# Polochon-street/bliss-rs

Measured on AMD Instinct MI355X. Metric: songs/sec (3-min 22 050 Hz f32) at 1/2/4/8 GPU; HBM GB/s vs roofline, higher is better.
Workload: dtype f32; 1 GPU; configs[1]: batch of 1024 synthetic 3969000-sample (3-min) white-noise f32 PCM buffers per GPU, full 23-feature descriptor set (FeaturesVersion 2); songs_per_gpu=1024, songs_total=1024, features=23, parallelism=single GPU

## Files before the change

bliss-rs_amd/csrc/ctx.hpp:

```cpp
#pragma once
#include <hip/hip_runtime.h>
#include <sched.h>

#include <map>
#include <memory>
#include <mutex>
#include <string>
#include <vector>

#include "../../include/blissgpu.h"
#include "internal.hpp"
#include "resample.hpp"
#include "staging_ring.hpp"

namespace bg {

int fail(int code, const char* what, const char* detail);

#define HIP_TRY(expr)                                                                           \
    do {                                                                                        \
        hipError_t e_ = (expr);                                                                 \
        if (e_ != hipSuccess) return ::bg::fail(BLISSGPU_ERR_HIP, #expr, hipGetErrorString(e_)); \
    } while (0)

struct EventPair { hipEvent_t a, b; };

template <typename T>
struct DevBuf {
    T* p = nullptr;
    size_t cap = 0;
    int ensure(size_t n) {
        if (n <= cap) return BLISSGPU_OK;
        if (p) (void)hipFree(p);
        p = nullptr;
        cap = 0;
        size_t want = n + n / 8 + 64;
        hipError_t e = hipMalloc((void**)&p, want * sizeof(T));
        if (e != hipSuccess && want > n) {
            (void)hipGetLastError();
            want = n;
            e = hipMalloc((void**)&p, want * sizeof(T));
        }
        if (e != hipSuccess) {
            (void)hipGetLastError();
            p = nullptr;
            return fail(BLISSGPU_ERR_OOM, "hipMalloc", hipGetErrorString(e));
        }
        cap = want;
        return BLISSGPU_OK;
    }
    void release() { if (p) (void)hipFree(p); p = nullptr; cap = 0; }
};

template <typename T>
struct PinnedBuf {
    T* p = nullptr;
    size_t cap = 0;
    int ensure(size_t n) {
        if (n <= cap) return BLISSGPU_OK;
        if (p) (void)hipHostFree(p);
        p = nullptr;
        cap = 0;
        const size_t want = n + n / 4 + 64;
        hipError_t e = hipHostMalloc((void**)&p, want * sizeof(T), hipHostMallocDefault);
        if (e != hipSuccess) { (void)hipGetLastError(); p = nullptr; return fail(BLISSGPU_ERR_OOM, "hipHostMalloc", hipGetErrorString(e)); }
        cap = want;
        return BLISSGPU_OK;
    }
    void release() { if (p) (void)hipHostFree(p); p = nullptr; cap = 0; }
};

struct ChunkSlot {
    DevBuf<uint8_t> slab;
    DevBuf<uint8_t> desc;
    PinnedBuf<uint8_t> h_desc;
    hipEvent_t ev_start = nullptr, ev_fork = nullptr, ev_stft = nullptr, ev_sel = nullptr, ev_tune = nullptr, ev_sum = nullptr, ev_chroma = nullptr;
    hipEvent_t ev_acf = nullptr, ev_beat = nullptr;
    bool beat_masked = false;
    static constexpr int MAX_PIECES = 8;
    hipEvent_t ev_piece[MAX_PIECES] = {};
    int pieces = 0;
    bg::SongRange piece[MAX_PIECES]{};
    hipEvent_t ev_desc = nullptr;
    hipEvent_t ev_free = nullptr;
    bool used = false;
    bool back_pending = false;
    Batch batch{};
    Workspace ws{};
};

#ifndef FEED_COPY_STREAMS
#define FEED_COPY_STREAMS 2
#endif
#ifndef STAGE_LANES_DEFAULT
#define STAGE_LANES_DEFAULT 4
#endif
#ifndef STAGE_SLABS_DEFAULT
#define STAGE_SLABS_DEFAULT 3
#endif
#ifndef STAGE_SLAB_KIB_DEFAULT
#define STAGE_SLAB_KIB_DEFAULT 4096
#endif
#ifndef STAGE_EVENT_FLAGS
#define STAGE_EVENT_FLAGS (hipEventDisableTiming | hipEventBlockingSync)
#endif
constexpr int N_COPY_STREAMS = FEED_COPY_STREAMS;
#ifndef FEED_BUFFERS
#define FEED_BUFFERS 3
#endif
constexpr int N_FEED_BUFFERS = FEED_BUFFERS;
constexpr uint32_t MAX_SAMPLE_RATE = 768000;
struct FeedSong {
    const void* p;
    uint64_t frames;
    uint32_t rate;
    uint8_t fmt;
    uint8_t channels;
    size_t frame_bytes() const { return (size_t)(fmt == BLISSGPU_SAMPLE_S16 ? 2 : 4) * channels; }
    bool direct() const { return fmt == BLISSGPU_SAMPLE_F32 && channels == 1 && rate == SWR_OUT_RATE; }
};
struct ResampleBank {
    SwrPlan plan;
    float* d_bank = nullptr;
    size_t bytes = 0;
    uint64_t last_use = 0;
};
#ifndef SWR_CACHE_BYTES
#define SWR_CACHE_BYTES (64ull << 20)
#endif

constexpr int MAX_STAGE_LANES = 16;
struct HipStageDev {
    int device;
    hipStream_t* streams;
    std::vector<int> cpus;
    void thread_begin(int) {
        (void)hipSetDevice(device);
        if (!cpus.empty()) {
            cpu_set_t set;
            CPU_ZERO(&set);
            for (int cpu : cpus)
                if (cpu >= 0 && cpu < CPU_SETSIZE) CPU_SET(cpu, &set);
            (void)sched_setaffinity(0, sizeof(set), &set);
        }
    }
    void* slab_alloc(size_t bytes) {
        void* p = nullptr;
        if (hipHostMalloc(&p, bytes, hipHostMallocDefault) != hipSuccess) { (void)hipGetLastError(); return nullptr; }
        return p;
    }
    void slab_free(void* p) { (void)hipHostFree(p); }
    void* event_create() {
        hipEvent_t e = nullptr;
        if (hipEventCreateWithFlags(&e, STAGE_EVENT_FLAGS) != hipSuccess) { (void)hipGetLastError(); return nullptr; }
        return (void*)e;
    }
    void event_destroy(void* e) { (void)hipEventDestroy((hipEvent_t)e); }
    int copy_async(void* dst, const void* slab, size_t bytes, int lane) {
        return (int)hipMemcpyAsync(dst, slab, bytes, hipMemcpyHostToDevice, streams[lane]);
    }
    int event_record(void* ev, int lane) { return (int)hipEventRecord((hipEvent_t)ev, streams[lane]); }
    int event_wait(void* ev) { return (int)hipEventSynchronize((hipEvent_t)ev); }
    std::string error_string(int code) { return hipGetErrorString((hipError_t)code); }
};

struct HostFeed {
    DevBuf<float> pcm[N_FEED_BUFFERS];
    DevBuf<uint8_t> raw[N_FEED_BUFFERS];
    DevBuf<float> out[N_FEED_BUFFERS];
    hipEvent_t ev_copied[N_FEED_BUFFERS][N_COPY_STREAMS] = {}, ev_done[N_FEED_BUFFERS] = {};
    hipStream_t copy_stream[N_COPY_STREAMS] = {};
    StageConfig stage_cfg{STAGE_LANES_DEFAULT, STAGE_SLABS_DEFAULT, (size_t)STAGE_SLAB_KIB_DEFAULT << 10};
    std::unique_ptr<StagingRing<HipStageDev>> ring;
    hipStream_t lane_stream[MAX_STAGE_LANES] = {};
    hipEvent_t ev_lane[N_FEED_BUFFERS][MAX_STAGE_LANES] = {};
    bool stage_numa = false;
    bool stage_numa_known = false;
    uint64_t staged_calls = 0;
    uint64_t staged_bytes = 0;
};

}

struct blissgpu_ctx {
    int device = 0;
    std::recursive_mutex mu;
    hipStream_t own_stream = nullptr;
    hipStream_t stream = nullptr;
    hipStream_t aux_stream = nullptr;
    hipStream_t chr_stream = nullptr;
    hipStream_t mask_stream = nullptr;
    int mask_cus = 0;
    int tail_mode = -1;
    uint32_t pipeline_chunks = 1;
    hipEvent_t ev_interop = nullptr;
    bool rolloff_exact_all = false;
    bool flux_order = false;
    int stft_shape = 0;
    int tail_split = 0;
    bool debug_chroma = false;
    bool serial = false;
    bool counted_live = false;
    uint64_t ws_limit = 0;
    uint32_t cand_budget = bg::CAND_BUDGET_PER_FRAME;
    float2 *tw8192 = nullptr, *tw512 = nullptr;
    float *hann8192 = nullptr, *hannz512 = nullptr, *bt_rwv = nullptr, *bt_dfwv = nullptr;
    double* chroma_bank = nullptr;
    bg::DeviceTables tables{};
    bg::ChunkSlot slot[2];
    uint64_t chunk_seq = 0;
    bg::DevBuf<int32_t> dbg_tuning;
    bg::DevBuf<uint32_t> dbg_nbpms;
    bg::DevBuf<double> dbg_chroma, dbg_interval;
    uint32_t dbg_n = 0;
    bg::Workspace last_ws{};
    std::vector<bg::SongDesc> last_songs;
    uint64_t last_chunks = 0;
    bg::HostFeed feed;
    std::map<uint32_t, bg::ResampleBank> swr_banks;
    size_t swr_bytes = 0;
    uint64_t swr_clock = 0;
    int64_t forest_split = 0;
    bool forest_global = false;
    int64_t forest_group_nodes = 0;
    bg::DevBuf<uint32_t> gf_img[2];
    bg::PinnedBuf<uint32_t> gf_host[2];
    hipEvent_t gf_ev[2] = {nullptr, nullptr};
    double gf_build_ms = 0.0, gf_wait_ms = 0.0;
    uint64_t gf_batches = 0;
    int n_cus = 0;
    bg::DevBuf<uint32_t> pl_sync, pl_keys;
    bg::DevBuf<uint32_t> pl_next;
    bg::DevBuf<uint8_t> pl_tmp;
    bg::DevBuf<unsigned long long> pl_slots;
    bg::DevBuf<uint8_t> pl_chain;
    bg::DevBuf<float> st_a, st_b, st_m, st_dist;
    bg::DevBuf<uint8_t> st_out;
    bg::DevBuf<uint32_t> st_idx;
// ... 64 lines not shown
```

bliss-rs_amd/csrc/kernels_chroma.hip:

```cpp
#include <float.h>
#include <stdlib.h>

#include <type_traits>

#include "device_utils.hpp"
#include "fft_r16.hpp"
#include "internal.hpp"

namespace bg {

typedef double double4_t __attribute__((ext_vector_type(4)));

__device__ __forceinline__ double tuning_of_slot(int slot) {
    return slot >= N_TUNING ? 0.0 : (-50.0 + (100.0 * 0.01 * (double)slot)) / 100.0;
}

__global__ __launch_bounds__(256) void chroma_bank_kernel(double* __restrict__ bank) {
#pragma clang fp contract(off)
    const int slot = blockIdx.y;
    const int k = blockIdx.x * 256 + threadIdx.x;
    if (k >= BANK_PITCH) return;
    double* out = bank + (size_t)slot * BANK_ROWS * BANK_PITCH;
    if (k >= CBINS) {
        for (int r = 0; r < BANK_ROWS; r++) out[(size_t)r * BANK_PITCH + k] = 0.0;
        return;
    }
    const double tuning = tuning_of_slot(slot);
    const double ncf = 12.0, nc2 = 6.0;
    const double step = 22050.0 / 8192.0;
    const double a440 = 440.0 * pow(2.0, tuning / 12.0);
    auto fbin = [&](int i) { return log2((0.0 + step * (double)i) / (a440 / 16.0)) * ncf; };
    const double fb1 = fbin(1);
    const double fb = (k == 0) ? fb1 - 1.5 * ncf : fbin(k);
    const double fbn = fbin(k + 1);
    double bw = fbn - fb;
    if (bw <= 1.0) bw = 1.0;
    double w[12], l2 = 0.0;
    for (int c = 0; c < 12; c++) {
        double d = -(double)c + fb;
        d = fmod(d + nc2 + 10.0 * ncf, ncf) - nc2;
        d = d / bw;
        w[c] = exp(-0.5 * (2.0 * d) * (2.0 * d));
        l2 += w[c] * w[c];
    }
    l2 = sqrt(l2);
    if (l2 < DBL_MIN) l2 = 1.0;
    const double y = (fb / ncf - 5.0) / 2.0;
    const double g = exp(-0.5 * (y * y));
    for (int r = 0; r < BANK_ROWS; r++) {
        double v = 0.0;
        if (r < 12) v = (w[(r + 3) % 12] / l2) * g;
        out[(size_t)r * BANK_PITCH + k] = v;
    }
}

void launch_chroma_bank(double* bank, hipStream_t st) {
    hipLaunchKernelGGL(chroma_bank_kernel, dim3((BANK_PITCH + 255) / 256, N_TUNING + 1), dim3(256), 0, st, bank);
}

__device__ __forceinline__ bool pip_is_peak(float sb, float se, float sa, double ref) {
    return (sa <= se) && (sb < se) && ((double)se > ref);
}

__device__ __forceinline__ void wave_append(bool is_peak, int c, uint16_t* list, uint32_t* count) {
    const uint64_t mask = __ballot(is_peak);
    if (mask == 0) return;
    const uint32_t lane = (uint32_t)lane_id();
    uint32_t base = 0;
    if (lane == 0) base = atomicAdd(count, (uint32_t)__popcll(mask));
    base = __shfl(base, 0, WAVE);
    if (is_peak) list[base + (uint32_t)__popcll(mask & ((1ull << lane) - 1ull))] = (uint16_t)c;
}

__device__ __forceinline__ bool pip_peak_core(float sb, float se, float sa, double ref, int c, double* mag_out,
                                              double* pitch_out) {
#pragma clang fp contract(off)
    if (!(sa <= se && sb < se)) return false;
    const double before = (double)sb, elem = (double)se, after = (double)sa;
    if (!(elem > ref)) return false;
    const double avg = 0.5 * (after - before);
    double shift = 2.0 * elem - after - before;
    if (fabs(shift) < DBL_MIN) shift += 1.0;
    shift = avg / shift;
    const double pitch = ((double)c + shift) * 22050.0 / 8192.0;
    if (!(pitch > 0.0)) return false;
    *mag_out = elem + 0.5 * avg * shift;
    *pitch_out = pitch;
    return true;
}

__device__ __forceinline__ bool pip_peak_mag(float sb, float se, float sa, double ref, int c, double* mag_out) {
    double pitch;
    return pip_peak_core(sb, se, sa, ref, c, mag_out, &pitch);
}

__device__ __forceinline__ int pitch_bin(double pitch) {
#pragma clang fp contract(off)
    double x = log2(pitch / (440.0 / 16.0));
    x = 12.0 * x;
    x = x - trunc(x);
    if (x >= 0.5) x -= 1.0;
    const double q = (x - -0.5) / 0.01;
    int idx = (q > 0.0) ? (int)q : 0;
    if (idx > N_TUNING - 1) idx = N_TUNING - 1;
    return idx;
}

__device__ __forceinline__ uint32_t coarse_bin(double mag) {
    const uint32_t b = __float_as_uint((float)mag) >> COARSE_SHIFT;
    return b < (uint32_t)H1_BINS ? b : (uint32_t)H1_BINS - 1;
}

__device__ __forceinline__ float ref_floor_f32(double ref) {
    float f = (float)ref;
    if ((double)f > ref) f = __uint_as_float(__float_as_uint(f) - 1u);
    return f;
}

__device__ __forceinline__ uint32_t peak_coarse_bin(float sb, float se, float sa, double ref, int c) {
    const float avg = 0.5f * (sa - sb);
    const float den = (2.0f * se - sa) - sb;
    const float shift = avg * __builtin_amdgcn_rcpf(den);
    const uint32_t bits = __float_as_uint(se + (0.5f * avg) * shift), low = bits & COARSE_LOW_MASK;
    if (se >= 1e-30f && low >= 16u && low <= COARSE_LOW_MASK - 16u) {
        const uint32_t b = bits >> COARSE_SHIFT;
        return b < (uint32_t)H1_BINS ? b : (uint32_t)H1_BINS - 1;
    }
    double mag;
    pip_peak_mag(sb, se, sa, ref, c, &mag);
    return coarse_bin(mag);
}

constexpr float PITCH_GUARD = 0.008f, PITCH_FLAT_LIMIT = 0.00390625f;
__device__ __forceinline__ int peak_pitch_bin_f32(float sb, float se, float sa, int c) {
    const float avg = 0.5f * (sa - sb);
    const float den = (2.0f * se - sa) - sb;
    if (!(se >= 1e-30f) || den < se * PITCH_FLAT_LIMIT) return -1;
    const float shift = avg * __builtin_amdgcn_rcpf(den);
    float x = 12.0f * (__builtin_amdgcn_logf((float)c + shift) + -3.3528687f);
    x = x - truncf(x);
    if (x >= 0.5f) x -= 1.0f;
    const float q = (x + 0.5f) * 100.0f;
    const float fl = floorf(q), fr = q - fl;
    if (fr < PITCH_GUARD || fr > 1.0f - PITCH_GUARD) return -1;
    const int idx = (int)fl;
    return idx < 0 ? 0 : (idx > N_TUNING - 1 ? N_TUNING - 1 : idx);
}

__device__ __attribute__((noinline)) uint32_t coarse_bin_exact(float sb, float se, float sa, double ref, int c) {
    double mag;
    pip_peak_mag(sb, se, sa, ref, c, &mag);
    return coarse_bin(mag);
}

__device__ __forceinline__ uint32_t peak_classify(float sb, float se, float sa, double ref, int c, int* pitch_bin_out) {
    const float avg = 0.5f * (sa - sb);
    const float den = (2.0f * se - sa) - sb;
    const float shift = avg * __builtin_amdgcn_rcpf(den);
    const bool normal = se >= 1e-30f;
    int pb = -1;
// ... 359 lines not shown
        __syncthreads();
        TRACE(16);
    }
    TRACE_FLUSH();
    if (have_base) {
        const uint32_t lbase = lhist_base;
        for (int i = t; i < LHIST_BINS; i += 256) {
            const uint32_t c = lhist[i];
            if (c) atomicAdd(&hist[lbase + i], c);
        }
    }
}

void launch_stft8192(const Batch& b, const Workspace& w, const DeviceTables& t, hipStream_t st, int shape) {
    if (b.tiles_c == 0) return;
    auto k = stft8192_kernel<false, false>;
    if (shape == 1) k = stft8192_kernel<true, true>;
    else if (shape == 2) k = stft8192_kernel<true, false>;
    else if (shape == 3) k = stft8192_kernel<false, true>;
    hipLaunchKernelGGL(k, dim3((b.tiles_c + 31u) & ~31u), dim3(256), 0, st,
                       b.pcm, b.songs, b.n_songs, b.pfx_c, t.hann8192, t.tw8192, w.spec, w.frame_max, w.h1, w.peak_rec, w.peak_cnt,
                       b.tiles_c);
}

__global__ __launch_bounds__(256) void tune_select_kernel(const SongDesc* __restrict__ songs,
                                                          const uint32_t* __restrict__ h1,
                                                          TuningState* __restrict__ tuning,
                                                          uint32_t* __restrict__ cand_cursor, uint32_t cand_pool,
                                                          uint32_t first_song) {
    __shared__ uint32_t wsum[4];
    __shared__ uint32_t s_total, s_blo, s_bhi;
    const uint32_t s = blockIdx.x + first_song;
    const int tid = threadIdx.x;
    TuningState* ts = tuning + s;
    auto no_peaks = [&]() {
        if (tid == 0) {
            ts->n_peaks = 0; ts->tuning_idx = -1; ts->n_cand = 0; ts->b_lo = 1; ts->b_hi = 0; ts->below = 0;
            ts->cand_off = 0; ts->cand_cap = 0;
        }
    };
    if (!songs[s].ok) { no_peaks(); return; }
    const uint32_t* hist = h1 + (size_t)s * H1_BINS;
    constexpr int PER = H1_BINS / 256;
    uint32_t local[PER], sum = 0;
#pragma unroll
    for (int i = 0; i < PER; i++) { local[i] = hist[tid * PER + i]; sum += local[i]; }
    const uint32_t incl = wave_scan_incl_u32(sum);
    if (lane_id() == 63) wsum[wave_id()] = incl;
    __syncthreads();
    uint32_t base = 0;
    for (int w = 0; w < wave_id(); w++) base += wsum[w];
    if (tid == 255) s_total = base + incl;
    __syncthreads();
    const uint32_t total = s_total;
    uint32_t before = base + incl - sum;
    if (total == 0) { no_peaks(); return; }
    const uint32_t r_lo = (total - 1) / 2, r_hi = total - 1 - r_lo;
    if (tid == 0) { ts->n_peaks = total; ts->n_cand = 0; ts->tuning_idx = -1; }
#pragma unroll
    for (int i = 0; i < PER; i++) {
        const uint32_t c = local[i];
        if (c) {
            if (before <= r_lo && r_lo < before + c) { ts->b_lo = tid * PER + i; ts->below = before; s_blo = tid * PER + i; }
            if (before <= r_hi && r_hi < before + c) { ts->b_hi = tid * PER + i; s_bhi = tid * PER + i; }
        }
        before += c;
    }
    __syncthreads();
    const uint32_t blo = s_blo, bhi = s_bhi;
    uint32_t mine = 0;
#pragma unroll
    for (int i = 0; i < PER; i++) {
        const uint32_t bin = tid * PER + i;
        if (bin >= blo && bin <= bhi) mine += local[i];
    }
    mine = wave_sum(mine);
    if (lane_id() == 0) wsum[wave_id()] = mine;
    __syncthreads();
    if (tid == 0) {
        const uint32_t want = wsum[0] + wsum[1] + wsum[2] + wsum[3];
        const uint32_t off = atomicAdd(cand_cursor, want);
        if (off <= cand_pool && want <= cand_pool - off) {
            ts->cand_off = off;
            ts->cand_cap = want;
        } else {
            atomicSub(cand_cursor, want);
            ts->cand_off = 0;
            ts->cand_cap = 0;
        }
    }
}

void launch_tune_select(const Batch& b, const Workspace& w, hipStream_t st, const SongRange* r) {
    const uint32_t s0 = r ? r->s0 : 0, s1 = r ? r->s1 : b.n_songs;
    if (s1 <= s0) return;
    hipLaunchKernelGGL(tune_select_kernel, dim3(s1 - s0), dim3(256), 0, st, b.songs, w.h1, w.tuning, w.cand_cursor,
                       w.cand_cap, s0);
}

constexpr int P2_SLOW_CAP = 1024;
constexpr int P2_FRAMES_PER_WAVE = CH_TILE / 4;

__global__ __launch_bounds__(256) void tune_pass2_kernel(const SongDesc* __restrict__ songs, uint32_t n_songs,
                                                         const uint32_t* __restrict__ pfx_ct,
                                                         const float* __restrict__ spec,
                                                         const float* __restrict__ frame_max,
                                                         const uint32_t* __restrict__ peak_rec,
                                                         const uint32_t* __restrict__ peak_cnt,
                                                         TuningState* __restrict__ tuning,
                                                         uint32_t* __restrict__ hist100,
                                                         double* __restrict__ cand_mag,
                                                         uint8_t* __restrict__ cand_pb, uint32_t first_tile) {
    __shared__ uint32_t hist[N_TUNING];
    __shared__ uint32_t slow_list[4][P2_SLOW_CAP];
    const uint32_t bx = blockIdx.x + first_tile;
    const uint32_t s = find_segment(pfx_ct, n_songs, bx);
    const SongDesc sd = songs[s];
    const uint32_t tile = bx - pfx_ct[s];
    const int tid = threadIdx.x, lane = lane_id(), wave = wave_id();
    TuningState* ts = tuning + s;
    const uint32_t b_lo = ts->b_lo, b_hi = ts->b_hi;
    if (ts->n_peaks == 0) return;
    const uint32_t cand_off = ts->cand_off;
    const uint32_t cand_cap = ts->cand_cap;
    const bool pooled = cand_cap != 0;
    if (tid < N_TUNING) hist[tid] = 0;
    __syncthreads();
    uint32_t n_slow = 0;

    auto flush = [&]() {
        for (uint32_t i = lane; i < n_slow; i += WAVE) {
            const uint32_t e = slow_list[wave][i];
            const int c = (int)(e & 0xFFFFu);
            const uint32_t f = tile * CH_TILE + wave + 4 * (e >> 16);
            const float* row = spec + (sd.c_off + f) * (size_t)CBINS_PAD;
            const double ref = 0.1 * (double)frame_max[sd.c_off + f];
            double mag, pitch;
            if (pip_peak_core(row[c - 1], row[c], row[c + 1], ref, c, &mag, &pitch)) {
                const uint32_t b = coarse_bin(mag);
                if (b > b_hi) {
                    atomicAdd(&hist[pitch_bin(pitch)], 1u);
                } else if (b >= b_lo) {
                    const uint32_t slot = atomicAdd(&ts->n_cand, 1u);
                    if (pooled && slot < cand_cap) {
                        cand_mag[cand_off + slot] = mag;
                        cand_pb[cand_off + slot] = (uint8_t)pitch_bin(pitch);
                    }
                }
            }
        }
        __builtin_amdgcn_wave_barrier();
        n_slow = 0;
    };
    uint32_t n_rec_next = 0;
    {
        const uint32_t f0 = tile * CH_TILE + wave;
        if (f0 < sd.n_c) n_rec_next = peak_cnt[sd.c_off + f0];
    }
    for (int i = 0; i < P2_FRAMES_PER_WAVE; i++) {
        const uint32_t f = tile * CH_TILE + wave + 4 * i;
        if (f >= sd.n_c) break;
        const uint32_t n_rec = n_rec_next < (uint32_t)PIP_MAX_PER_FRAME ? n_rec_next : (uint32_t)PIP_MAX_PER_FRAME;
        if (i + 1 < P2_FRAMES_PER_WAVE && f + 4 < sd.n_c) n_rec_next = peak_cnt[sd.c_off + f + 4];
        const uint32_t* __restrict__ recs = peak_rec + (sd.c_off + f) * (size_t)PIP_MAX_PER_FRAME;
        if (n_slow + PIP_MAX_PER_FRAME > P2_SLOW_CAP) flush();
        for (uint32_t j0 = 0; j0 < n_rec; j0 += 4 * WAVE) {
            uint32_t r4[4];
#pragma unroll
            for (int u = 0; u < 4; u++) {
                const uint32_t j = j0 + WAVE * u + lane;
                r4[u] = j < n_rec ? recs[j] : 0xFFFFFFFFu;
            }
#pragma unroll
            for (int u = 0; u < 4; u++) {
                if (j0 + WAVE * u >= n_rec) break;
                const uint32_t j = j0 + WAVE * u + lane;
                bool slow = false;
                uint32_t c = 0;
                if (j < n_rec) {
                    const uint32_t r = r4[u];
                    const uint32_t b = r >> 18, pbf = (r >> 11) & 0x7Fu;
                    c = r & 0x7FFu;
                    if (b > b_hi) {
                        if (pbf) atomicAdd(&hist[pbf - 1], 1u);
                        else slow = true;
                    } else if (b >= b_lo) {
                        slow = true;
                    }
                }
                const uint64_t mask = __ballot(slow);
                if (mask) {
                    if (slow) slow_list[wave][n_slow + (uint32_t)__popcll(mask & ((1ull << lane) - 1ull))] = ((uint32_t)i << 16) | c;
                    n_slow += (uint32_t)__popcll(mask);
                }
            }
        }
    }
    __builtin_amdgcn_wave_barrier();
    flush();
    __syncthreads();
    if (tid < N_TUNING && hist[tid]) atomicAdd(&hist100[(size_t)s * N_TUNING + tid], hist[tid]);
}

void launch_tune_pass2(const Batch& b, const Workspace& w, hipStream_t st, const SongRange* r) {
    const uint32_t t0 = r ? r->ct0 : 0, t1 = r ? r->ct1 : b.tiles_ct;
    if (t1 <= t0) return;
    hipLaunchKernelGGL(tune_pass2_kernel, dim3(t1 - t0), dim3(256), 0, st, b.songs, b.n_songs, b.pfx_ct, w.spec,
                       w.frame_max, w.peak_rec, w.peak_cnt, w.tuning, w.hist100, w.cand_mag, w.cand_pb, t0);
}

template <typename ForEach>
__device__ uint64_t block_radix_select(ForEach&& for_each, uint32_t rank, uint32_t* hist, uint32_t* s_digit, uint32_t* s_rank,
                                       uint32_t* s_wave) {
    const int tid = threadIdx.x;
    uint64_t prefix = 0, mask = 0;
    for (int shift = 56; shift >= 0; shift -= 8) {
        hist[tid] = 0;
        __syncthreads();
        for_each([&](double mag, int) {
            const uint64_t k = f64_key(mag);
            const bool in = (k & mask) == prefix;
            const uint32_t d = (uint32_t)(k >> shift) & 0xFFu;
            const uint64_t m = __ballot(in);
            if (m != 0) {
                const int first = __ffsll((unsigned long long)m) - 1;
                const uint32_t d0 = (uint32_t)__shfl((int)d, first, WAVE);
                if (__ballot(in && d == d0) == m) {
                    if (lane_id() == first) atomicAdd(&hist[d0], (uint32_t)__popcll(m));
                } else if (in) {
                    atomicAdd(&hist[d], 1u);
                }
            }
        });
        __syncthreads();
        {
            const uint32_t h = hist[tid];
            const uint32_t incl = wave_scan_incl_u32(h);
            if (lane_id() == 63) s_wave[wave_id()] = incl;
            __syncthreads();
            uint32_t below = incl - h;
            for (int w = 0; w < wave_id(); w++) below += s_wave[w];
            if (h != 0 && below <= rank && rank < below + h) {
                *s_digit = (uint32_t)tid;
                *s_rank = rank - below;
            }
        }
        __syncthreads();
        prefix |= (uint64_t)(*s_digit) << shift;
        mask |= 0xFFull << shift;
        rank = *s_rank;
        __syncthreads();
    }
    return prefix;
}

__global__ __launch_bounds__(256) void tune_final_kernel(const SongDesc* __restrict__ songs,
                                                         TuningState* __restrict__ tuning,
                                                         const uint32_t* __restrict__ hist100,
                                                         const double* __restrict__ cand_mag,
                                                         const uint8_t* __restrict__ cand_pb,
                                                         const float* __restrict__ spec,
                                                         const float* __restrict__ frame_max,
                                                         const uint32_t* __restrict__ peak_rec,
                                                         const uint32_t* __restrict__ peak_cnt, uint32_t first_song) {
    __shared__ uint32_t hist[256];
    __shared__ uint32_t s_digit, s_rank, s_cnt_le, s_wave[4];
    __shared__ unsigned long long s_min_gt;
    const uint32_t s = blockIdx.x + first_song;
    const int tid = threadIdx.x;
    TuningState* ts = tuning + s;
    const SongDesc sd = songs[s];
    if (!sd.ok || ts->n_peaks == 0) return;
    const uint32_t total = ts->n_peaks, nc = ts->n_cand;
    const uint32_t r_lo = (total - 1) / 2, r_hi = total - 1 - r_lo;
    const uint32_t k_lo = r_lo - ts->below, k_hi = r_hi - ts->below;
    const uint32_t b_lo = ts->b_lo, b_hi = ts->b_hi;
    const bool pooled = ts->cand_cap != 0 && nc == ts->cand_cap;
    const double* v = cand_mag + ts->cand_off;
    const uint8_t* pb = cand_pb + ts->cand_off;

    auto for_each = [&](auto&& fn) {
        if (pooled) {
            for (uint32_t i0 = tid; i0 < nc; i0 += 8 * 256) {
                double m8[8];
                int b8[8];
#pragma unroll
                for (int u = 0; u < 8; u++) {
                    const uint32_t i = i0 + 256u * u;
                    m8[u] = i < nc ? v[i] : 0.0;
                    b8[u] = i < nc ? (int)pb[i] : 0;
                }
#pragma unroll
                for (int u = 0; u < 8; u++)
                    if (i0 + 256u * u < nc) fn(m8[u], b8[u]);
            }
        } else {
            for (uint32_t f = 0; f < sd.n_c; f++) {
                const uint32_t n_rec_raw = peak_cnt[sd.c_off + f];
                const uint32_t n_rec = n_rec_raw < (uint32_t)PIP_MAX_PER_FRAME ? n_rec_raw : (uint32_t)PIP_MAX_PER_FRAME;
                const uint32_t* __restrict__ recs = peak_rec + (sd.c_off + f) * (size_t)PIP_MAX_PER_FRAME;
                const float* __restrict__ row = spec + (sd.c_off + f) * (size_t)CBINS_PAD;
                const double ref = 0.1 * (double)frame_max[sd.c_off + f];
                for (uint32_t j = tid; j < n_rec; j += 256) {
                    const uint32_t r = recs[j], b = r >> 18;
                    if (b < b_lo || b > b_hi) continue;
                    const int c = (int)(r & 0x7FFu);
                    double mag, pitch;
                    if (pip_peak_core(row[c - 1], row[c], row[c + 1], ref, c, &mag, &pitch)) fn(mag, pitch_bin(pitch));
                }
            }
        }
    };

    const uint64_t key_lo = block_radix_select(for_each, k_lo, hist, &s_digit, &s_rank, s_wave);
    uint64_t key_hi = key_lo;
    if (k_hi != k_lo) {
        if (tid == 0) { s_cnt_le = 0; s_min_gt = ~0ull; }
        __syncthreads();
        uint32_t cnt = 0;
        unsigned long long mn = ~0ull;
        for_each([&](double mag, int) {
            const uint64_t k = f64_key(mag);
            if (k <= key_lo) cnt++;
            else if (k < mn) mn = k;
        });
        atomicAdd(&s_cnt_le, cnt);
        atomicMin(&s_min_gt, mn);
        __syncthreads();
        if (s_cnt_le <= k_hi) key_hi = s_min_gt;
    }
    double thr;
    {
#pragma clang fp contract(off)
        const double lo = key_f64(key_lo), hi = key_f64(key_hi);
        thr = lo + (hi - lo) / 2.0;
    }
    __syncthreads();
    if (tid < N_TUNING) hist[tid] = hist100[(size_t)s * N_TUNING + tid];
    __syncthreads();
    for_each([&](double mag, int bin) {
        if (mag >= thr) atomicAdd(&hist[bin], 1u);
    });
    __syncthreads();
    if (tid == 0) {
        uint32_t best = 0;
        for (uint32_t k = 1; k < N_TUNING; k++)
            if (hist[k] > hist[best]) best = k;
        ts->tuning_idx = (int32_t)best;
// ... 165 lines not shown
```

bliss-rs_amd/csrc/scheduler.hip:

```cpp
#include <string.h>

#include <algorithm>
#include <chrono>
#include <condition_variable>
#include <numeric>

#include "coalescing_front.hpp"
#include "ctx.hpp"

using namespace bg;

namespace {

inline size_t align_up(size_t x, size_t a) { return (x + a - 1) / a * a; }

void fill_counts(SongDesc& d) {
    const uint64_t n = d.n;
    d.n_t = (uint32_t)((n - W512) / HOP_T + 1);
    d.n_b = (uint32_t)((n - W512) / HOP_B + 1);
    d.n_f = std::max(d.n_t, 2u * d.n_b);
    d.n_c = (uint32_t)ceilf((float)n / (float)HOP_C);
    d.n_e = (uint32_t)((n + 255) / 256);
    d.n_l = (uint32_t)((n + LOUD_W - 1) / LOUD_W);
}

size_t song_ws_bytes(const SongDesc& d) {
    if (!d.ok) return 256;
    size_t b = 0;
    b += (size_t)d.n_t * 12 + (size_t)d.n_b * 8 + (size_t)d.n_e * 8;
    b += (size_t)d.n_c * (CBINS_PAD * 4 + 4);
    b += (size_t)H1_BINS * 4 + N_TUNING * 4 + sizeof(TuningState) + sizeof(TempoState);
    b += (size_t)d.n_c * CAND_BUDGET_PER_FRAME * 9;
    b += (size_t)d.n_c * (PIP_MAX_PER_FRAME * 4 + 4);
    b += ((size_t)d.n_c / CH_TILE + 1) * 80;
    b += ((size_t)d.n_b / BT_STEP + 2) * (8 + BT_PRE_STRIDE * 4);
    return b + 4096;
}

struct Carver {
    uint8_t* base;
    size_t off = 0;
    template <typename T>
    T* take(size_t n) {
        off = align_up(off, 256);
        T* p = reinterpret_cast<T*>(base + off);
        off += n * sizeof(T);
        return p;
    }
};

struct ChunkTotals {
    uint64_t tot_t = 0, tot_b = 0, tot_c = 0, tot_e = 0;
    uint32_t max_nb = 0, max_nt = 0, max_runs = 1;
    uint32_t tiles_ct = 0;
    uint64_t cand_cap = 0;
};

Workspace carve(uint8_t* base, uint32_t ns, const ChunkTotals& t, size_t* bytes) {
    Carver m{base};
    Workspace w{};
    w.centroid = m.take<float>(t.tot_t); w.rolloff = m.take<float>(t.tot_t); w.flatness = m.take<float>(t.tot_t);
    w.flux = m.take<float>(t.tot_b); w.thresholded = m.take<float>(t.tot_b);
    w.e256 = m.take<float>(t.tot_e); w.zc256 = m.take<uint32_t>(t.tot_e);
    static_assert((size_t)(CBINS_PAD + PIP_MAX_PER_FRAME) * 4 * HOP_T >= (size_t)256 * 4 * HOP_C,
                  "the borrowed stretch must hold one 256-word entry per timbral frame: bytes per chroma frame x samples per "
                  "timbral frame >= bytes per entry x samples per chroma frame");
    w.spec = m.take<float>(t.tot_c * CBINS_PAD + 64);
    w.peak_rec = m.take<uint32_t>(t.tot_c * PIP_MAX_PER_FRAME);
    w.roll_fix_bytes = (size_t)(reinterpret_cast<uint8_t*>(w.peak_rec + t.tot_c * PIP_MAX_PER_FRAME) - reinterpret_cast<uint8_t*>(w.spec));
    w.frame_max = m.take<float>(t.tot_c);
    w.roll_fix = m.take<RollFix>(1);
    w.h1 = m.take<uint32_t>((size_t)ns * H1_BINS); w.hist100 = m.take<uint32_t>((size_t)ns * N_TUNING);
    w.tuning = m.take<TuningState>(ns);
    w.peak_cnt = m.take<uint32_t>(t.tot_c);
    w.cand_mag = m.take<double>(t.cand_cap); w.cand_pb = m.take<uint8_t>(t.cand_cap);
    w.cand_cursor = m.take<uint32_t>(4);
    w.cand_cap = (uint32_t)t.cand_cap;
    w.chroma_part = m.take<double>((size_t)t.tiles_ct * 10 + 16);
    w.tempo = m.take<TempoState>(ns);
    w.run_bpm = m.take<float>((size_t)ns * t.max_runs); w.run_cnt = m.take<uint32_t>((size_t)ns * t.max_runs);
    w.runs_pitch = t.max_runs;
    w.bt_pre = m.take<float>((size_t)(t.tot_b / BT_STEP + ns + 1) * BT_PRE_STRIDE);
    w.summary = m.take<float>((size_t)ns * 16);
    *bytes = m.off + 4096;
    return w;
}

int ensure_mask_stream(blissgpu_ctx* c, int cus) {
    cus = std::max(1, std::min(cus, c->n_cus));
    if (c->mask_stream && c->mask_cus == cus) return BLISSGPU_OK;
    if (c->mask_stream) { (void)hipStreamSynchronize(c->mask_stream); (void)hipStreamDestroy(c->mask_stream); c->mask_stream = nullptr; }
    std::vector<uint32_t> mask((size_t)(c->n_cus + 31) / 32, 0u);
    for (int i = 0; i < cus; i++) mask[(size_t)i / 32] |= 1u << (i % 32);
    HIP_TRY(hipExtStreamCreateWithCUMask(&c->mask_stream, (uint32_t)mask.size(), mask.data()));
    c->mask_cus = cus;
    return BLISSGPU_OK;
}

int ensure_slot_events(ChunkSlot& s) {
    if (s.ev_free) return BLISSGPU_OK;
    hipEvent_t* evs[] = {&s.ev_start, &s.ev_fork, &s.ev_stft, &s.ev_sel, &s.ev_tune, &s.ev_sum, &s.ev_chroma, &s.ev_desc, &s.ev_free, &s.ev_acf, &s.ev_beat};
    for (hipEvent_t* e : evs) HIP_TRY(hipEventCreateWithFlags(e, hipEventDisableTiming));
    for (hipEvent_t& e : s.ev_piece) HIP_TRY(hipEventCreateWithFlags(&e, hipEventDisableTiming));
    return BLISSGPU_OK;
}

int chunk_front(blissgpu_ctx* c, ChunkSlot& slot, const float* d_pcm, SongDesc* songs, uint32_t ns, bool only_chunk) {
    int rc = ensure_slot_events(slot);
    if (rc) return rc;
    std::vector<uint32_t> pfx_f(ns + 1, 0), pfx_c(ns + 1, 0), pfx_ct(ns + 1, 0), pfx_cw(ns + 1, 0);
    ChunkTotals t;
    for (uint32_t i = 0; i < ns; i++) {
        SongDesc& d = songs[i];
        d.t_off = t.tot_t; d.b_off = t.tot_b; d.c_off = t.tot_c; d.e_off = t.tot_e;
        if (d.ok) {
            t.tot_t += d.n_t; t.tot_b += d.n_b; t.tot_c += d.n_c; t.tot_e += d.n_e;
            t.max_nb = std::max(t.max_nb, d.n_b);
            t.max_nt = std::max(t.max_nt, d.n_t);
            t.max_runs = std::max(t.max_runs, d.n_b / BT_STEP + 1);
        }
        pfx_f[i + 1] = pfx_f[i] + (d.ok ? (d.n_f + F512_TILE - 1) / F512_TILE : 0);
        pfx_c[i + 1] = pfx_c[i] + (d.ok ? 4 * ((d.n_c + 4 * STFT_TILE - 1) / (4 * STFT_TILE)) : 0);
        pfx_ct[i + 1] = pfx_ct[i] + (d.ok ? (d.n_c + CH_TILE - 1) / CH_TILE : 0);
        pfx_cw[i + 1] = pfx_cw[i] + (d.ok ? (d.n_c + 4 * CH_TILE - 1) / (4 * CH_TILE) : 0);
    }
    t.tiles_ct = pfx_ct[ns];
    t.cand_cap = std::min<uint64_t>(t.tot_c * (uint64_t)c->cand_budget, 0xFFFFFF00ull) + 64;

    const size_t desc_bytes = align_up(ns * sizeof(SongDesc), 256) + 4 * align_up((ns + 1) * 4, 256) + 256;
    size_t need = 0;
    (void)carve(nullptr, ns, t, &need);
    if ((rc = slot.desc.ensure(desc_bytes))) return rc;
    if ((rc = slot.slab.ensure(need))) return rc;
    if (slot.used) HIP_TRY(hipEventSynchronize(slot.ev_desc));
    if ((rc = slot.h_desc.ensure(desc_bytes))) return rc;

    hipStream_t st = c->stream, sb = c->serial ? c->stream : c->aux_stream, sc = c->serial ? c->stream : c->chr_stream;
    const bool multi = !c->serial;
    if (slot.used && multi) HIP_TRY(hipStreamWaitEvent(st, slot.ev_free, 0));

    uint8_t* h = slot.h_desc.p;
    size_t o = 0;
    const size_t o_songs = o; memcpy(h + o, songs, ns * sizeof(SongDesc)); o = align_up(o + ns * sizeof(SongDesc), 256);
    const size_t o_f = o; memcpy(h + o, pfx_f.data(), (ns + 1) * 4); o = align_up(o + (ns + 1) * 4, 256);
    const size_t o_c = o; memcpy(h + o, pfx_c.data(), (ns + 1) * 4); o = align_up(o + (ns + 1) * 4, 256);
    const size_t o_ct = o; memcpy(h + o, pfx_ct.data(), (ns + 1) * 4); o = align_up(o + (ns + 1) * 4, 256);
    const size_t o_cw = o; memcpy(h + o, pfx_cw.data(), (ns + 1) * 4); o = align_up(o + (ns + 1) * 4, 256);
    HIP_TRY(hipMemcpyAsync(slot.desc.p, h, o, hipMemcpyHostToDevice, st));
    slot.used = true;

    Batch& b = slot.batch;
    b = Batch{};
    b.pcm = d_pcm;
    b.songs = reinterpret_cast<const SongDesc*>(slot.desc.p + o_songs);
    b.n_songs = ns;
    b.pfx_f = reinterpret_cast<const uint32_t*>(slot.desc.p + o_f);
    b.pfx_c = reinterpret_cast<const uint32_t*>(slot.desc.p + o_c);
    b.pfx_ct = reinterpret_cast<const uint32_t*>(slot.desc.p + o_ct);
    b.pfx_cw = reinterpret_cast<const uint32_t*>(slot.desc.p + o_cw);
    b.tiles_f = pfx_f[ns]; b.tiles_c = pfx_c[ns]; b.tiles_ct = pfx_ct[ns]; b.tiles_cw = pfx_cw[ns];
    b.total_b = t.tot_b; b.max_nb = t.max_nb; b.max_nt = t.max_nt;

    size_t used_bytes = 0;
    slot.ws = carve(slot.slab.p, ns, t, &used_bytes);
    slot.ws.dbg_chroma = nullptr;
    slot.ws.dbg_interval = nullptr;
    if (c->debug_chroma) {
        if ((rc = c->dbg_chroma.ensure((size_t)t.tot_c * 12 + 12))) return rc;
        if ((rc = c->dbg_interval.ensure((size_t)ns * 10))) return rc;
        slot.ws.dbg_chroma = c->dbg_chroma.p;
        slot.ws.dbg_interval = c->dbg_interval.p;
    }
    const Workspace& w = slot.ws;
    c->last_ws = w;
    c->last_songs.assign(songs, songs + ns);
    {
        RollFix rf{};
        if ((uint64_t)w.roll_fix_bytes / (256 * 4) < t.tot_t)
            return fail(BLISSGPU_ERR_INVALID, "chunk_front", "internal: the borrowed stretch cannot hold one exact-rolloff entry per timbral frame");
        rf.cap = (uint32_t)t.tot_t;
        rf.mags = w.spec;
        memcpy(h + o, &rf, sizeof(rf));
        HIP_TRY(hipMemcpyAsync(w.roll_fix, h + o, sizeof(rf), hipMemcpyHostToDevice, st));
    }
    HIP_TRY(hipEventRecord(slot.ev_desc, st));

    HIP_TRY(hipMemsetAsync(w.h1, 0, (size_t)ns * H1_BINS * 4, st));
    HIP_TRY(hipMemsetAsync(w.hist100, 0, (size_t)ns * N_TUNING * 4, st));
    HIP_TRY(hipMemsetAsync(w.cand_cursor, 0, 16, st));
    { Prof p(c, K_FFT512); launch_fft512(b, w, c->tables, st, c->rolloff_exact_all, c->flux_order); }
    { Prof p(c, K_ROLLFIX); launch_rolloff_fix(b, w, t.tot_t, st); }
    if (multi) {
        HIP_TRY(hipEventRecord(slot.ev_fork, st));
        HIP_TRY(hipStreamWaitEvent(sb, slot.ev_fork, 0));
    }
    { Prof p(c, K_ONSET, sb); launch_onset(b, w, sb); }
    { Prof p(c, K_SUMMARY, sb); launch_summary(b, w, sb); }
    slot.beat_masked = multi && c->tail_mode >= 2;
    if (slot.beat_masked) {
        if ((rc = ensure_mask_stream(c, c->tail_mode))) return rc;
        { Prof p(c, K_BEAT, sb); launch_beat_acf(b, w, c->tables, sb); }
        HIP_TRY(hipEventRecord(slot.ev_acf, sb));
        HIP_TRY(hipStreamWaitEvent(c->mask_stream, slot.ev_acf, 0));
        { Prof p(c, K_BEAT, c->mask_stream); launch_beat_track(b, w, c->tables, c->mask_stream); }
        HIP_TRY(hipEventRecord(slot.ev_beat, c->mask_stream));
    }
    const bool acf_early = multi && c->tail_mode == -2;
    if (acf_early) { Prof p(c, K_BEAT, sb); launch_beat_acf(b, w, c->tables, sb); }
    const bool beat_last = multi && c->tail_mode == -3;
    const bool beat_late = !slot.beat_masked && !beat_last && (c->tail_mode == 1 || acf_early || (c->tail_mode < 0 && only_chunk));
    if (!beat_late && !slot.beat_masked && !beat_last) { Prof p(c, K_BEAT, sb); launch_beat(b, w, c->tables, sb); }
    { Prof p(c, K_STFT8192); launch_stft8192(b, w, c->tables, st, c->stft_shape); }
    if (multi) {
        HIP_TRY(hipEventRecord(slot.ev_stft, st));
        HIP_TRY(hipStreamWaitEvent(sc, slot.ev_stft, 0));
    }
    slot.pieces = 0;
    if (multi && only_chunk && c->tail_split > 1 && ns >= 2) {
        const int want = std::min<int>(std::min<int>(c->tail_split, ChunkSlot::MAX_PIECES), (int)ns);
        uint32_t s0 = 0;
        for (int k = 0; k < want && s0 < ns; k++) {
            uint32_t s1 = s0 + 1;
            const uint64_t goal = (uint64_t)pfx_ct[ns] * (uint64_t)(k + 1) / (uint64_t)want;
            while (s1 < ns && (k == want - 1 || pfx_ct[s1] < goal)) s1++;
            slot.piece[slot.pieces++] = SongRange{s0, s1, pfx_ct[s0], pfx_ct[s1], pfx_cw[s0], pfx_cw[s1]};
            s0 = s1;
        }
        if (slot.pieces < 2) slot.pieces = 0;
    }
    if (slot.pieces) {
        for (int k = 0; k < slot.pieces; k++) {
            { Prof p(c, K_TUNE_SELECT, sc); launch_tune_select(b, w, sc, &slot.piece[k]); }
            if (k == 1 && beat_late) {
                HIP_TRY(hipEventRecord(slot.ev_sel, sc));
                HIP_TRY(hipStreamWaitEvent(sb, slot.ev_sel, 0));
                Prof p(c, K_BEAT, sb);
                if (acf_early) launch_beat_track(b, w, c->tables, sb); else launch_beat(b, w, c->tables, sb);
            }
            { Prof p(c, K_TUNE_PASS2, sc); launch_tune_pass2(b, w, sc, &slot.piece[k]); }
            { Prof p(c, K_TUNE_FINAL, sc); launch_tune_final(b, w, sc, &slot.piece[k]); }
            HIP_TRY(hipEventRecord(slot.ev_piece[k], sc));
        }
        if (beat_last) {
            HIP_TRY(hipStreamWaitEvent(sb, slot.ev_piece[slot.pieces - 1], 0));
            Prof p(c, K_BEAT, sb);
            launch_beat(b, w, c->tables, sb);
        }
        HIP_TRY(hipGetLastError());
        slot.back_pending = true;
        return BLISSGPU_OK;
    }
    { Prof p(c, K_TUNE_SELECT, sc); launch_tune_select(b, w, sc); }
    if (beat_late) {
        if (multi) {
            HIP_TRY(hipEventRecord(slot.ev_sel, sc));
            HIP_TRY(hipStreamWaitEvent(sb, slot.ev_sel, 0));
        }
        Prof p(c, K_BEAT, sb);
        if (acf_early) launch_beat_track(b, w, c->tables, sb); else launch_beat(b, w, c->tables, sb);
    }
    { Prof p(c, K_TUNE_PASS2, sc); launch_tune_pass2(b, w, sc); }
    { Prof p(c, K_TUNE_FINAL, sc); launch_tune_final(b, w, sc); }
    if (multi) HIP_TRY(hipEventRecord(slot.ev_tune, sc));
    if (beat_last) {
        HIP_TRY(hipStreamWaitEvent(sb, slot.ev_tune, 0));
        Prof p(c, K_BEAT, sb);
        launch_beat(b, w, c->tables, sb);
    }
    HIP_TRY(hipGetLastError());
    slot.back_pending = true;
    return BLISSGPU_OK;
}

int chunk_back(blissgpu_ctx* c, ChunkSlot& slot, uint32_t features_version, float* d_out, int32_t* d_status) {
    if (!slot.back_pending) return BLISSGPU_OK;
    slot.back_pending = false;
    hipStream_t st = c->stream, sb = c->serial ? c->stream : c->aux_stream;
    const bool multi = !c->serial;
    if (slot.pieces) {
        for (int k = 0; k < slot.pieces; k++) {
            HIP_TRY(hipStreamWaitEvent(st, slot.ev_piece[k], 0));
            Prof p(c, K_CHROMA);
            launch_chroma(slot.batch, slot.ws, c->tables, st, &slot.piece[k]);
        }
    } else {
        if (multi) HIP_TRY(hipStreamWaitEvent(st, slot.ev_tune, 0));
        Prof p(c, K_CHROMA);
        launch_chroma(slot.batch, slot.ws, c->tables, st);
    }
    if (multi) {
        HIP_TRY(hipEventRecord(slot.ev_chroma, st));
        HIP_TRY(hipStreamWaitEvent(sb, slot.ev_chroma, 0));
        if (slot.beat_masked) HIP_TRY(hipStreamWaitEvent(sb, slot.ev_beat, 0));
    }
    { Prof p(c, K_FINALIZE, sb); launch_finalize(slot.batch, slot.ws, features_version, d_out, d_status, c->dbg_tuning.p, c->dbg_nbpms.p, sb); }
    if (multi) HIP_TRY(hipEventRecord(slot.ev_free, sb));
    HIP_TRY(hipGetLastError());
    return BLISSGPU_OK;
}

}

namespace bg {

void scheduler_release(blissgpu_ctx* c) {
    for (ChunkSlot& s : c->slot) {
        s.slab.release(); s.desc.release(); s.h_desc.release();
        hipEvent_t evs[] = {s.ev_start, s.ev_fork, s.ev_stft, s.ev_sel, s.ev_tune, s.ev_sum, s.ev_chroma, s.ev_desc, s.ev_free, s.ev_acf, s.ev_beat};
        for (hipEvent_t e : evs)
            if (e) (void)hipEventDestroy(e);
        for (hipEvent_t e : s.ev_piece)
            if (e) (void)hipEventDestroy(e);
        s = ChunkSlot{};
    }
    HostFeed& f = c->feed;
    f.ring.reset();
    for (hipStream_t& ls : f.lane_stream)
        if (ls) { (void)hipStreamSynchronize(ls); (void)hipStreamDestroy(ls); ls = nullptr; }
    for (auto& row : f.ev_lane)
        for (hipEvent_t& ev : row)
            if (ev) { (void)hipEventDestroy(ev); ev = nullptr; }
    for (auto& kv : c->swr_banks)
        if (kv.second.d_bank) (void)hipFree(kv.second.d_bank);
    c->swr_banks.clear();
    c->swr_bytes = 0;
    for (hipStream_t& cs : f.copy_stream)
        if (cs) { (void)hipStreamSynchronize(cs); (void)hipStreamDestroy(cs); cs = nullptr; }
    for (int b = 0; b < N_FEED_BUFFERS; b++) {
        f.pcm[b].release(); f.raw[b].release(); f.out[b].release();
        for (hipEvent_t& ev : f.ev_copied[b])
            if (ev) { (void)hipEventDestroy(ev); ev = nullptr; }
        if (f.ev_done[b]) (void)hipEventDestroy(f.ev_done[b]);
        f.ev_done[b] = nullptr;
    }
}

#ifndef FEED_GROUP_MIB
#define FEED_GROUP_MIB 512
#endif
#ifndef FEED_GROUP_PCM_FACTOR
#define FEED_GROUP_PCM_FACTOR 1
#endif
#ifndef STAGE_MIN_BYTES
#define STAGE_MIN_BYTES (8ull << 20)
#endif
int resample_bank(blissgpu_ctx* c, uint32_t rate, const ResampleBank** out, const char* who) {
    auto it = c->swr_banks.find(rate);
    if (it == c->swr_banks.end()) {
        ResampleBank rb;
        if (rate > MAX_SAMPLE_RATE || !swr_make_plan(rate, &rb.plan))
            return fail(BLISSGPU_ERR_INVALID, who, "sample_rate must be 1 .. 768000 Hz");
        std::vector<float> bank;
        swr_make_filter(rb.plan, bank);
        rb.bytes = bank.size() * sizeof(float);
        while (!c->swr_banks.empty() && c->swr_bytes + rb.bytes > (size_t)SWR_CACHE_BYTES) {
            auto lru = c->swr_banks.begin();
            for (auto q = c->swr_banks.begin(); q != c->swr_banks.end(); ++q)
                if (q->second.last_use < lru->second.last_use) lru = q;
            if (lru->second.d_bank) (void)hipFree(lru->second.d_bank);
            c->swr_bytes -= lru->second.bytes;
            c->swr_banks.erase(lru);
        }
        float* d = nullptr;
        hipError_t e = hipMalloc((void**)&d, rb.bytes);
        if (e != hipSuccess) { (void)hipGetLastError(); return fail(BLISSGPU_ERR_OOM, "hipMalloc(resample bank)", hipGetErrorString(e)); }
        e = hipMemcpy(d, bank.data(), rb.bytes, hipMemcpyHostToDevice);
        if (e != hipSuccess) { (void)hipFree(d); return fail(BLISSGPU_ERR_HIP, "hipMemcpy(resample bank)", hipGetErrorString(e)); }
        rb.d_bank = d;
        c->swr_bytes += rb.bytes;
        it = c->swr_banks.emplace(rate, rb).first;
    }
    it->second.last_use = ++c->swr_clock;
    *out = &it->second;
    return BLISSGPU_OK;
}

std::vector<int> parse_cpulist(const char* text) {
    std::vector<int> cpus;
    for (const char* p = text; p && *p;) {
        char* end = nullptr;
        const long a = strtol(p, &end, 10);
        if (end == p || a < 0) break;
        long b = a;
        if (*end == '-') {
            const char* q = end + 1;
            b = strtol(q, &end, 10);
            if (end == q || b < a) break;
        }
        for (long v = a; v <= b && cpus.size() < 4096; v++) cpus.push_back((int)v);
        p = *end == ',' ? end + 1 : end;
        if (*end != ',') break;
    }
    return cpus;
}

std::vector<int> device_local_cpus(int device) {
    char bus[32] = {0};
    if (hipDeviceGetPCIBusId(bus, (int)sizeof(bus), device) != hipSuccess) { (void)hipGetLastError(); return {}; }
    for (char* p = bus; *p; p++) *p = (char)tolower((unsigned char)*p);
    const std::string base = std::string("/sys/bus/pci/devices/") + bus;
    char line[4096] = {0};
    int node = -1;
    if (FILE* f = fopen((base + "/numa_node").c_str(), "r")) {
        if (fgets(line, sizeof(line), f)) node = atoi(line);
        fclose(f);
    }
    if (node < 0) return {};
    std::vector<int> cpus;
    if (FILE* f = fopen((base + "/local_cpulist").c_str(), "r")) {
        if (fgets(line, sizeof(line), f)) cpus = parse_cpulist(line);
        fclose(f);
    }
    return cpus;
}

int enqueue_decode(blissgpu_ctx* c, const void* d_in, int fmt, uint32_t channels, uint64_t frames, uint32_t rate, float* d_out,
                   uint64_t n_out, hipStream_t st, const char* who) {
    if (rate == SWR_OUT_RATE) {
        launch_pcm_convert(d_in, fmt, channels, d_out, frames, st);
        HIP_TRY(hipGetLastError());
        return BLISSGPU_OK;
    }
    const ResampleBank* rb;
    const int rc = resample_bank(c, rate, &rb, who);
    if (rc) return rc;
    HIP_TRY(launch_resample(d_in, fmt, channels, frames, rb->plan, rb->d_bank, d_out, n_out, st));
    return BLISSGPU_OK;
}

int analyze_host_songs(blissgpu_ctx* c, const FeedSong* in, uint32_t n_songs, uint32_t features_version, float* out,
                       int32_t* status, const char* who, float* d_rows) {
    const uint32_t d = blissgpu_feature_count(features_version);
    if (!d) return fail(BLISSGPU_ERR_INVALID, who, "features_version must be 1 or 2");
    if (n_songs == 0) return BLISSGPU_OK;
    std::vector<uint64_t> out_len(n_songs);
    bool any_raw = false;
    for (uint32_t i = 0; i < n_songs; i++) {
        const FeedSong& fs = in[i];
        if (fs.channels == 0 || fs.channels > 8) return fail(BLISSGPU_ERR_INVALID, who, "channels must be 1..8");
        if (fs.fmt != BLISSGPU_SAMPLE_F32 && fs.fmt != BLISSGPU_SAMPLE_S16 && fs.fmt != BLISSGPU_SAMPLE_S32)
            return fail(BLISSGPU_ERR_INVALID, who, "sample_format must be F32, S16 or S32");
        if (fs.rate == 0 || fs.rate > MAX_SAMPLE_RATE) return fail(BLISSGPU_ERR_INVALID, who, "sample_rate must be 1 .. 768000 Hz");
        if (fs.frames && !fs.p) return fail(BLISSGPU_ERR_INVALID, who, "NULL song pointer");
        if (fs.rate == SWR_OUT_RATE) out_len[i] = fs.frames;
        else {
            SwrPlan pl;
            swr_make_plan(fs.rate, &pl);
            out_len[i] = swr_out_len(pl, fs.frames);
        }
// ... 544 lines not shown
```

Baseline: 28380 songs/sec.

## Vectorize tune pass-2 record loads and rebalance memsets/finalize across streams

The tuning pass-2 kernel now fetches peak records as 8-byte pairs, so each lane classifies two records per load and there are fewer load instructions. It also reads all per-frame counts with one lane-parallel load and broadcasts them with readlane instead of prefetching serially. In the single-chunk multi-stream case, the zeroing memsets move to the aux stream so they overlap the FFT work, and finalize runs on the main stream after chroma without a cross-stream hop. This adds event dependencies, and the 8-byte loads rely on each row staying 8-byte aligned.

```diff
diff --git a/bliss-rs_amd/csrc/ctx.hpp b/bliss-rs_amd/csrc/ctx.hpp
--- a/bliss-rs_amd/csrc/ctx.hpp
+++ b/bliss-rs_amd/csrc/ctx.hpp
@@ -84,6 +84,8 @@
     hipEvent_t ev_desc = nullptr;
     hipEvent_t ev_free = nullptr;
     bool used = false;
+    bool only_chunk = false;
+    bool fill_aux = false;
     bool back_pending = false;
     Batch batch{};
     Workspace ws{};
diff --git a/bliss-rs_amd/csrc/kernels_chroma.hip b/bliss-rs_amd/csrc/kernels_chroma.hip
--- a/bliss-rs_amd/csrc/kernels_chroma.hip
+++ b/bliss-rs_amd/csrc/kernels_chroma.hip
@@ -6,6 +6,7 @@
 #include "device_utils.hpp"
 #include "fft_r16.hpp"
 #include "internal.hpp"
+#include "tune_fetch.hpp"
 
 namespace bg {
 
@@ -671,33 +672,35 @@
         __builtin_amdgcn_wave_barrier();
         n_slow = 0;
     };
-    uint32_t n_rec_next = 0;
-    {
-        const uint32_t f0 = tile * CH_TILE + wave;
-        if (f0 < sd.n_c) n_rec_next = peak_cnt[sd.c_off + f0];
-    }
-    for (int i = 0; i < P2_FRAMES_PER_WAVE; i++) {
-        const uint32_t f = tile * CH_TILE + wave + 4 * i;
-        if (f >= sd.n_c) break;
-        const uint32_t n_rec = n_rec_next < (uint32_t)PIP_MAX_PER_FRAME ? n_rec_next : (uint32_t)PIP_MAX_PER_FRAME;
-        if (i + 1 < P2_FRAMES_PER_WAVE && f + 4 < sd.n_c) n_rec_next = peak_cnt[sd.c_off + f + 4];
-        const uint32_t* __restrict__ recs = peak_rec + (sd.c_off + f) * (size_t)PIP_MAX_PER_FRAME;
-        if (n_slow + PIP_MAX_PER_FRAME > P2_SLOW_CAP) flush();
-        for (uint32_t j0 = 0; j0 < n_rec; j0 += 4 * WAVE) {
-            uint32_t r4[4];
-#pragma unroll
-            for (int u = 0; u < 4; u++) {
-                const uint32_t j = j0 + WAVE * u + lane;
-                r4[u] = j < n_rec ? recs[j] : 0xFFFFFFFFu;
-            }
-#pragma unroll
-            for (int u = 0; u < 4; u++) {
-                if (j0 + WAVE * u >= n_rec) break;
-                const uint32_t j = j0 + WAVE * u + lane;
+    static_assert(TF_ROW_WORDS == (uint32_t)PIP_MAX_PER_FRAME && TF_LANES == (uint32_t)WAVE, "tune_fetch.hpp restates these");
+    const uint32_t f0 = tile * CH_TILE + wave;
+    const uint32_t n_frames = f0 < sd.n_c ? min((uint32_t)P2_FRAMES_PER_WAVE, (sd.n_c - f0 + 3u) / 4u) : 0u;
+    uint32_t cnt_lane = 0;
+    if ((uint32_t)lane < n_frames) cnt_lane = peak_cnt[sd.c_off + f0 + 4u * (uint32_t)lane];
+    auto count_of = [&](uint32_t i) {
+        const uint32_t n = (uint32_t)__builtin_amdgcn_readlane((int)cnt_lane, (int)i);
+        return n < (uint32_t)PIP_MAX_PER_FRAME ? n : (uint32_t)PIP_MAX_PER_FRAME;
+    };
+    auto row_of = [&](uint32_t i) { return peak_rec + (sd.c_off + f0 + 4u * i) * (size_t)PIP_MAX_PER_FRAME; };
+    auto fetch = [&](uint2 (&r)[TF_LOADS], const uint32_t* __restrict__ recs, uint32_t round, uint32_t n_rec) {
+#pragma unroll
+        for (uint32_t u = 0; u < TF_LOADS; u++) {
+            uint2 v = make_uint2(TF_FILLER, TF_FILLER);
+            if (tf_load_issued(round, u, (uint32_t)lane, n_rec))
+                v = *reinterpret_cast<const uint2*>(recs + tf_record_index(round, u, (uint32_t)lane, 0));
+            r[u] = v;
+        }
+    };
+    auto classify = [&](const uint2 (&r4)[TF_LOADS], uint32_t round, uint32_t n_rec, uint32_t i) {
+#pragma unroll
+        for (uint32_t u = 0; u < TF_LOADS; u++) {
+            if (tf_record_index(round, u, 0, 0) >= n_rec) break;
+#pragma unroll
+            for (uint32_t half = 0; half < TF_PAIR; half++) {
                 bool slow = false;
                 uint32_t c = 0;
-                if (j < n_rec) {
-                    const uint32_t r = r4[u];
+                if (tf_valid(round, u, (uint32_t)lane, half, n_rec)) {
+                    const uint32_t r = half ? r4[u].y : r4[u].x;
                     const uint32_t b = r >> 18, pbf = (r >> 11) & 0x7Fu;
                     c = r & 0x7FFu;
                     if (b > b_hi) {
@@ -709,10 +712,20 @@
                 }
                 const uint64_t mask = __ballot(slow);
                 if (mask) {
-                    if (slow) slow_list[wave][n_slow + (uint32_t)__popcll(mask & ((1ull << lane) - 1ull))] = ((uint32_t)i << 16) | c;
+                    if (slow) slow_list[wave][n_slow + (uint32_t)__popcll(mask & ((1ull << lane) - 1ull))] = (i << 16) | c;
                     n_slow += (uint32_t)__popcll(mask);
                 }
             }
+        }
+    };
+    for (uint32_t i = 0; i < n_frames; i++) {
+        const uint32_t n_rec = count_of(i);
+        const uint32_t* __restrict__ recs = row_of(i);
+        if (n_slow + PIP_MAX_PER_FRAME > P2_SLOW_CAP) flush();
+        for (uint32_t round = 0; round < tf_rounds(n_rec); round++) {
+            uint2 r4[TF_LOADS];
+            fetch(r4, recs, round, n_rec);
+            classify(r4, round, n_rec, i);
         }
     }
     __builtin_amdgcn_wave_barrier();
diff --git a/bliss-rs_amd/csrc/scheduler.hip b/bliss-rs_amd/csrc/scheduler.hip
--- a/bliss-rs_amd/csrc/scheduler.hip
+++ b/bliss-rs_amd/csrc/scheduler.hip
@@ -108,6 +108,7 @@
 int chunk_front(blissgpu_ctx* c, ChunkSlot& slot, const float* d_pcm, SongDesc* songs, uint32_t ns, bool only_chunk) {
     int rc = ensure_slot_events(slot);
     if (rc) return rc;
+    slot.only_chunk = only_chunk;
     std::vector<uint32_t> pfx_f(ns + 1, 0), pfx_c(ns + 1, 0), pfx_ct(ns + 1, 0), pfx_cw(ns + 1, 0);
     ChunkTotals t;
     for (uint32_t i = 0; i < ns; i++) {
@@ -137,7 +138,8 @@
 
     hipStream_t st = c->stream, sb = c->serial ? c->stream : c->aux_stream, sc = c->serial ? c->stream : c->chr_stream;
     const bool multi = !c->serial;
-    if (slot.used && multi) HIP_TRY(hipStreamWaitEvent(st, slot.ev_free, 0));
+    const bool had_prev = slot.used;
+    if (had_prev && multi) HIP_TRY(hipStreamWaitEvent(st, slot.ev_free, 0));
 
     uint8_t* h = slot.h_desc.p;
     size_t o = 0;
@@ -185,9 +187,15 @@
     }
     HIP_TRY(hipEventRecord(slot.ev_desc, st));
 
-    HIP_TRY(hipMemsetAsync(w.h1, 0, (size_t)ns * H1_BINS * 4, st));
-    HIP_TRY(hipMemsetAsync(w.hist100, 0, (size_t)ns * N_TUNING * 4, st));
-    HIP_TRY(hipMemsetAsync(w.cand_cursor, 0, 16, st));
+    slot.fill_aux = multi && only_chunk;
+    {
+        hipStream_t sf = slot.fill_aux ? sb : st;
+        if (slot.fill_aux && had_prev) HIP_TRY(hipStreamWaitEvent(sf, slot.ev_free, 0));
+        HIP_TRY(hipMemsetAsync(w.h1, 0, (size_t)ns * H1_BINS * 4, sf));
+        HIP_TRY(hipMemsetAsync(w.hist100, 0, (size_t)ns * N_TUNING * 4, sf));
+        HIP_TRY(hipMemsetAsync(w.cand_cursor, 0, 16, sf));
+        if (slot.fill_aux) HIP_TRY(hipEventRecord(slot.ev_start, sf));
+    }
     { Prof p(c, K_FFT512); launch_fft512(b, w, c->tables, st, c->rolloff_exact_all, c->flux_order); }
     { Prof p(c, K_ROLLFIX); launch_rolloff_fix(b, w, t.tot_t, st); }
     if (multi) {
@@ -210,6 +218,7 @@
     const bool beat_last = multi && c->tail_mode == -3;
     const bool beat_late = !slot.beat_masked && !beat_last && (c->tail_mode == 1 || acf_early || (c->tail_mode < 0 && only_chunk));
     if (!beat_late && !slot.beat_masked && !beat_last) { Prof p(c, K_BEAT, sb); launch_beat(b, w, c->tables, sb); }
+    if (slot.fill_aux) HIP_TRY(hipStreamWaitEvent(st, slot.ev_start, 0));
     { Prof p(c, K_STFT8192); launch_stft8192(b, w, c->tables, st, c->stft_shape); }
     if (multi) {
         HIP_TRY(hipEventRecord(slot.ev_stft, st));
@@ -288,13 +297,19 @@
         Prof p(c, K_CHROMA);
         launch_chroma(slot.batch, slot.ws, c->tables, st);
     }
-    if (multi) {
+    const bool on_main = multi && slot.only_chunk;
+    if (on_main) {
+        HIP_TRY(hipEventRecord(slot.ev_sum, sb));
+        HIP_TRY(hipStreamWaitEvent(st, slot.ev_sum, 0));
+        if (slot.beat_masked) HIP_TRY(hipStreamWaitEvent(st, slot.ev_beat, 0));
+    } else if (multi) {
         HIP_TRY(hipEventRecord(slot.ev_chroma, st));
         HIP_TRY(hipStreamWaitEvent(sb, slot.ev_chroma, 0));
         if (slot.beat_masked) HIP_TRY(hipStreamWaitEvent(sb, slot.ev_beat, 0));
     }
-    { Prof p(c, K_FINALIZE, sb); launch_finalize(slot.batch, slot.ws, features_version, d_out, d_status, c->dbg_tuning.p, c->dbg_nbpms.p, sb); }
-    if (multi) HIP_TRY(hipEventRecord(slot.ev_free, sb));
+    hipStream_t sf = on_main ? st : sb;
+    { Prof p(c, K_FINALIZE, sf); launch_finalize(slot.batch, slot.ws, features_version, d_out, d_status, c->dbg_tuning.p, c->dbg_nbpms.p, sf); }
+    if (multi) HIP_TRY(hipEventRecord(slot.ev_free, sf));
     HIP_TRY(hipGetLastError());
     return BLISSGPU_OK;
 }
diff --git a/bliss-rs_amd/csrc/tune_fetch.hpp b/bliss-rs_amd/csrc/tune_fetch.hpp
--- /dev/null
+++ b/bliss-rs_amd/csrc/tune_fetch.hpp
@@ -0,0 +1,34 @@
+#pragma once
+#include <cstdint>
+
+namespace bg {
+
+constexpr uint32_t TF_LANES = 64;
+constexpr uint32_t TF_LOADS = 4;
+constexpr uint32_t TF_PAIR = 2;
+constexpr uint32_t TF_PER_LOAD = TF_LANES * TF_PAIR;
+constexpr uint32_t TF_PER_ROUND = TF_PER_LOAD * TF_LOADS;
+constexpr uint32_t TF_ROW_WORDS = 714;
+constexpr uint32_t TF_FILLER = 0xFFFFFFFFu;
+
+constexpr uint32_t tf_rounds(uint32_t n_rec) { return (n_rec + TF_PER_ROUND - 1) / TF_PER_ROUND; }
+
+constexpr uint32_t tf_record_index(uint32_t round, uint32_t u, uint32_t lane, uint32_t half) {
+    return round * TF_PER_ROUND + u * TF_PER_LOAD + lane * TF_PAIR + half;
+}
+
+constexpr bool tf_load_issued(uint32_t round, uint32_t u, uint32_t lane, uint32_t n_rec) {
+    return tf_record_index(round, u, lane, 0) < n_rec;
+}
+constexpr bool tf_valid(uint32_t round, uint32_t u, uint32_t lane, uint32_t half, uint32_t n_rec) {
+    return tf_record_index(round, u, lane, half) < n_rec;
+}
+
+constexpr uint64_t tf_load_byte_offset(uint64_t row, uint32_t round, uint32_t u, uint32_t lane) {
+    return (row * TF_ROW_WORDS + tf_record_index(round, u, lane, 0)) * 4u;
+}
+
+static_assert(TF_ROW_WORDS % TF_PAIR == 0, "a pair must not straddle two rows");
+static_assert((TF_ROW_WORDS * 4u) % 8u == 0, "every row starts 8-byte aligned");
+
+}
```

After: 28570 songs/sec, median of 6. About the same (+0.7%).
